# HKUNLP/efficient-attention

Hardware: AMD Instinct MI355X
Metric: attn fwd+bwd tokens/s per GPU at N=784, d=64; 1/2/4/8-GPU DDP scaling (higher is better)
Workload: dtype bf16; 1 GPU; lara attention layer fwd+bwd+SGD, x=[128,28,28,192] per GPU (N=784, h=3, d=64), bf16 autocast; attn=lara, global_batch=128, seq_len=784, heads=3, head_dim=64, parallelism=dp1, hipgraph=True, gemm_tunableop=False

## Files before the change

efficient-attention_amd/build.py:

```python
#!/usr/bin/env python3
import glob
import os
import subprocess
import sys

HERE = os.path.dirname(os.path.abspath(__file__))
CSRC = os.path.join(HERE, "csrc")
LIBDIR = os.path.join(HERE, "lib")
INCLUDE = os.path.join(os.path.dirname(HERE), "include")
HIPCC = os.environ.get("HIPCC", "/opt/rocm/bin/hipcc")
FLAGS = ["--offload-arch=gfx950", "-O3", "-std=c++17", "-fPIC", "-mllvm", "-amdgpu-mfma-vgpr-form", "-I" + INCLUDE, "-I" + CSRC]

LIB_SOURCES = ["ea_capi.hip", "ea_window_fwd.hip", "ea_window_bwd.hip", "ea_eva_landmark.hip",
               "ea_lara_x.hip", "ea_lara_y.hip", "ea_lara_f.hip", "ea_softmax.hip",
               "ea_lara_merge.hip", "ea_proj.hip", "ea_lara_segment.hip",
               "ea_rows_mlp.hip", "ea_wgrad.hip", "ea_linear.hip", "ea_lmk2.hip", "ea_scatter.hip", "ea_proj_rs.hip",
               "ea_performer_f32.hip", "ea_fold.hip", "ea_lara_seglin.hip", "ea_layernorm.hip", "ea_dgrad_rs.hip", "ea_f32_attn.hip",
               "ea_kernelized.hip", "ea_ceva_decode.hip", "ea_ceva_decode_linear.hip", "ea_ceva_decode_vocab.hip", "ea_lara_xp.hip",
               "ea_vocab_score.hip", "ea_adaptive_score.hip", "ea_adaptive_pick.hip", "ea_vocab_nll.hip", "ea_adaptive_nll.hip"]


def _cuid(src):
    return "-cuid=" + os.path.splitext(src)[0]


def _newer(target, deps):
    if not os.path.exists(target):
        return True
    t = os.path.getmtime(target)
    return any(os.path.getmtime(d) > t for d in deps)


def _run(cmd):
    r = subprocess.run(cmd, stdout=subprocess.PIPE, stderr=subprocess.STDOUT, text=True)
    if r.returncode != 0:
        raise RuntimeError("build failed: %s\n%s" % (" ".join(cmd), r.stdout))
    return r.stdout


def build(force=False, verbose=False):
    os.makedirs(LIBDIR, exist_ok=True)
    headers = glob.glob(os.path.join(CSRC, "*.h")) + glob.glob(os.path.join(INCLUDE, "*.h"))
    objs, jobs = [], []
    for src in LIB_SOURCES:
        s = os.path.join(CSRC, src)
        o = os.path.join(LIBDIR, src.replace(".hip", ".o"))
        if force or _newer(o, [s] + headers):
            if verbose:
                print("hipcc -c", src, flush=True)
            jobs.append([HIPCC] + FLAGS + [_cuid(src), "-c", s, "-o", o])
        objs.append(o)
    if jobs:
# ... 55 lines not shown
```

efficient-attention_amd/csrc/ea_capi.hip:

```cpp
#include <stdlib.h>
#include <cmath>
#include "ea_window.h"
#include "ea_landmark_params.h"
#include "ea_lara.h"
#include "ea_softmax.h"
#include "ea_lara_lmk.h"
#include "ea_lara_merge.h"
#include "ea_layernorm.h"
#include "ea_lara_segment.h"
#include "ea_scatter.h"
#include "ea_rows_mlp.h"
#include "ea_performer_f32.h"
#include "ea_kernelized.h"
#include "ea_f32_tile.h"
#include "ea_f32_attn.h"
#include "ea_linear.h"
#include "ea_proj.h"
#include "ea_fold.h"
#include "ea_lara_seglin.h"

using namespace ea;

static bool t4_ok32(const ea_t4* t, int D, int N) {
  return view_ok(t, D, 2) && (int64_t)N * t->sn < ((int64_t)1 << 31);
// ... 1326 lines not shown
  if ((dpq == nullptr) != (dpk == nullptr)) return EA_E_BADARG;
  if (dpq && (pool_r <= 0 || gh % pool_r || gw % pool_r)) return EA_E_BADARG;
  if (uq && (!qkv || !qbar || !lse_t || ldq < 192 || (ldq & 7) || C <= 0)) return EA_E_BADARG;
  if (uq && C > 64) return EA_E_UNSUPPORTED;
  if (!uq && !dpq) return EA_E_BADARG;
  if ((int64_t)B * gh * gw >= ((int64_t)1 << 31)) return EA_E_BADARG;
  return dgrad_fin_launch(dtype, dqkv, (long)ldy, qkv, (long)ldq, w, w_f32, dx, dx_f32, (long)ldx, B, gh, gw, pool_r, C, scale,
                          qbar, uq, lse_t, dpq, dpk, (hipStream_t)stream);
}

int32_t ea_linear_pool_supported(int32_t in_features, int32_t out_features, int32_t B, int32_t gh, int32_t gw, int32_t r) {
  return proj_rs_pool_supported(in_features, out_features, B, gh, gw, r);
}

int ea_linear_w32_pool(int32_t dtype, int32_t B, int32_t gh, int32_t gw, int32_t r, int32_t in_features, int32_t out_features,
                       const void* a, int32_t a_f32, int64_t lda, const float* w, const float* bias, void* y, int64_t ldy,
                       void* a_cast, float* pooled_q, float* pooled_k, void* w_cast, void* stream) {
  if (!a || !w || !y || !pooled_q || !pooled_k || ((uintptr_t)a & 15) || ((uintptr_t)w & 15) || ((uintptr_t)y & 15) ||
      ((uintptr_t)bias & 15) || ((uintptr_t)a_cast & 15) || ((uintptr_t)pooled_q & 15) || ((uintptr_t)pooled_k & 15) ||
      ((uintptr_t)w_cast & 15))
    return EA_E_BADARG;
  if (lda < in_features || ldy < out_features || (lda & 7) || (ldy & 7)) return EA_E_BADARG;
  if (!proj_rs_pool_supported(in_features, out_features, B, gh, gw, r)) return EA_E_UNSUPPORTED;
  return proj_rs_dispatch(dtype, a, a_f32, w, bias, y, a_cast, B * gh * gw, (long)lda, (long)ldy, (hipStream_t)stream, B, gh, gw,
                          r, pooled_q, pooled_k, w_cast, nullptr);
}

int ea_linear_w192_prepare(int32_t dtype, const float* wq, const float* wp, void* w16q, void* wq_sw, void* w16p, void* w16pT,
                           void* stream) {
  if (!wq || !w16q || !wq_sw || ((uintptr_t)wq & 15) || ((uintptr_t)wp & 15) || ((uintptr_t)w16q & 15) || ((uintptr_t)wq_sw & 15) ||
      ((uintptr_t)w16p & 15) || ((uintptr_t)w16pT & 15))
    return EA_E_BADARG;
  if (wp && (!w16p || !w16pT)) return EA_E_BADARG;
  return w192_prepare_dispatch(dtype, wq, wp, w16q, wq_sw, w16p, w16pT, nullptr, (hipStream_t)stream);
}

int ea_linear_w192_prepare_t(int32_t dtype, const float* wq, const float* wp, void* w16q, void* wq_sw, void* w16p, void* w16pT,
                             void* wqT_sw, void* stream) {
  if (!wq || !w16q || !wq_sw || !wqT_sw || ((uintptr_t)wq & 15) || ((uintptr_t)wp & 15) || ((uintptr_t)w16q & 15) ||
      ((uintptr_t)wq_sw & 15) || ((uintptr_t)w16p & 15) || ((uintptr_t)w16pT & 15) || ((uintptr_t)wqT_sw & 15))
    return EA_E_BADARG;
  if (wp && (!w16p || !w16pT)) return EA_E_BADARG;
  return w192_prepare_dispatch(dtype, wq, wp, w16q, wq_sw, w16p, w16pT, wqT_sw, (hipStream_t)stream);
}

int ea_linear_wsw(int32_t dtype, int32_t rows, int32_t B, int32_t gh, int32_t gw, int32_t r, const void* a, int32_t a_f32, int64_t lda,
                  const void* wq_sw, const float* bias, void* y, int64_t ldy, void* a_cast, float* pooled_q, float* pooled_k,
                  void* stream) {
  if (!a || !wq_sw || !y || ((uintptr_t)a & 15) || ((uintptr_t)wq_sw & 15) || ((uintptr_t)y & 15) || ((uintptr_t)bias & 15) ||
      ((uintptr_t)a_cast & 15) || ((uintptr_t)pooled_q & 15) || ((uintptr_t)pooled_k & 15))
    return EA_E_BADARG;
  if (lda < 192 || ldy < 576 || (lda & 7) || (ldy & 7) || rows <= 0) return EA_E_BADARG;
  if (r != 0) {
    if (!pooled_q || !pooled_k || rows != B * gh * gw) return EA_E_BADARG;
    if (!proj_rs_pool_supported(192, 576, B, gh, gw, r)) return EA_E_UNSUPPORTED;
  }
  return proj_rs_dispatch(dtype, a, a_f32, nullptr, bias, y, a_cast, rows, (long)lda, (long)ldy, (hipStream_t)stream, B, gh, gw, r,
                          r ? pooled_q : nullptr, r ? pooled_k : nullptr, nullptr, wq_sw);
}

}

static int fill_sb(const ea_sb_geom* g, SbP& p) {
  if (!g || g->B <= 0 || g->H <= 0 || g->N <= 0 || g->window <= 0 || (g->dtype != EA_BF16 && g->dtype != EA_F16))
    return EA_E_BADARG;
  if (g->D != 64 || g->M <= 0 || g->M > 64) return EA_E_UNSUPPORTED;
  p.B = g->B; p.H = g->H; p.N = g->N; p.M = g->M; p.w = g->window;
  p.G.N = g->N; p.G.attn2d = g->attn_2d; p.G.gh = g->attn_2d ? g->gh : 1; p.G.gw = g->attn_2d ? g->gw : g->N;
  if (g->attn_2d) {
    if (g->gh % g->window || g->gw % g->window || g->gh * g->gw != g->N) return EA_E_BADARG;
    p.Wq = g->window * g->window;
    p.nwin = (g->gh / g->window) * (g->gw / g->window);
  } else {
    if (g->N % g->window) return EA_E_BADARG;
    p.Wq = g->window;
    p.nwin = g->N / g->window;
// ... 1427 lines not shown
```

efficient-attention_amd/csrc/ea_linear.h:

```cpp
#pragma once
#include "ea_common.h"

namespace ea {

int linear_supported(int K, int NO);
int proj_rs_supported(int K, int NO);
int proj_rs_pool_supported(int K, int NO, int B, int gh, int gw, int r);
int proj_rs_dispatch(int dtype, const void* a, int a_f32, const float* w, const float* bias, void* y, void* a_cast, int rows,
                     long lda, long ldy, hipStream_t st, int B, int gh, int gw, int r, float* pq, float* pk, void* w_cast,
                     const void* wsw);
int w192_prepare_dispatch(int dtype, const float* wq, const float* wp, void* w16q, void* wsw, void* w16p, void* w16pT, void* wtsw,
                          hipStream_t st);
int dgrad_rs_supported(int K, int NO);
int dgrad_fin_launch(int dtype, const void* dqkv, long ldy, const void* qkv, long ldq, const void* w, int w_f32, void* dx, int dx_f32,
                     long ldx, int B, int gh, int gw, int pool_r, int C, float scale, const float* qbar, const float* uq,
                     const float* lse_t, const float* dpq, const float* dpk, hipStream_t st);
int dgrad_rs_dispatch(int dtype, const void* dy, const void* w, int w_f32, void* dx, int dx_f32, int rows, long ldy, long ldx,
                      hipStream_t st);
int linear_dispatch(int dtype, const void* a, int a_f32, const void* w, int w_mode, const float* bias, void* y, int y_f32,
                    void* a_cast, int rows, int K, int NO, long lda, long ldy, hipStream_t st);
int wgrad_slices(int rows, int M, int K);
int wgrad_pair_slices(int rows, int M1, int K1, int M2, int K2);
int wgrad_pair_dispatch(int dtype, int rows, const void* dy1, const void* x1, float* part1, float* db1, long ld1, int M1, int K1,
                        const void* dy2, const void* x2, float* part2, float* db2, long ld2, int M2, int K2, hipStream_t st);
int wgrad_dispatch(int dtype, const void* dy, const void* x, float* part, float* db_part, long part_ld, int rows, int M,
                   int K, hipStream_t st);
int part_sum_dispatch(const float* part, float* out, int S, int n, long ld, hipStream_t st);
int multi_sum_dispatch(int K, const float* const* part, const int* S, const int* n, const long long* ld, float* const* out,
                       hipStream_t st);

}
```

efficient-attention_amd/csrc/ea_proj_rs.hip:

```cpp
#include "ea_common.h"
#include "ea_linear.h"

namespace ea {

struct RsP {
  const char* a;
  const float* w;
  const float* bias;
  char* y;
  char* a_cast;
  char* w_cast;
  int rows, ntiles;
  long lda, ldy;
  float *pq, *pk;
  int gw, cw, Lc, ntok, ncell;
  unsigned m_Lc, m_cw;
  long long* prof;
  const char* wsw;
};

constexpr int RS_K = 192, RS_NO = 576, RS_WAVES = 12, RS_TOK = 32, RS_KT = RS_K / 32, RS_SLABS = RS_K / 64;

EA_DEV int rs_off(int slab, int tok, int chunk16) { return slab * (RS_TOK * 128) + lds_off3<64>(tok, chunk16); }

// ... 177 lines not shown
      const u32x4 o = {third[0][0], third[0][1], third[1][0], third[1][1]};
      stg16(p.y + ((size_t)tok * p.ldy + c0 + 32 + 8 * (g >> 1)) * 2, o);
    }
#ifndef EA_RS_NOPOOLMATH
    if constexpr (POOL > 0) {
      if (tprev >= 0) pool_out(tprev, buf ^ 1);
    }
#endif
  }
  EA_BLKX(p, 1);
  if constexpr (POOL > 0) {
    if (tprev >= 0) {
      __syncthreads();
      pool_out(tprev, buf ^ 1);
    }
  }
  EA_BLK(p, 1);
}

int proj_rs_supported(int K, int NO) { return K == RS_K && NO == RS_NO; }

static unsigned rs_magic(int d) { return (unsigned)((1ull << 32) / (unsigned)d) + 1u; }

int proj_rs_pool_supported(int K, int NO, int B, int gh, int gw, int r) {
  if (K != RS_K || NO != RS_NO || (r != 2 && r != 4) || B <= 0 || gh <= 0 || gw <= 0 || gh % r || gw % r) return 0;
  const long Lc = (long)(gh / r) * (gw / r), ncell = (long)B * Lc;
  return ncell * Lc < (1l << 32) && (long)B * gh * gw < (1l << 31);
}

template <typename E>
__global__ __launch_bounds__(256) void w192_prepare_kernel(const float* __restrict__ wq, const float* __restrict__ wp,
                                                            char* __restrict__ w16q, char* __restrict__ wsw,
                                                            char* __restrict__ w16p, char* __restrict__ w16pT,
                                                            char* __restrict__ wtsw) {
  constexpr int NQ = RS_WAVES * 3 * RS_KT * 64, NP = RS_K * RS_K / 8, NT = 12 * (RS_NO / 32) * 64;
  const int i = blockIdx.x * 256 + threadIdx.x;
  if (i < NQ) {
    const int lane = i & 63, pc = i >> 6, ks = pc % RS_KT, wj = pc / RS_KT, j = wj % 3, wave = wj / 3;
    const int g = lane >> 4, li = lane & 15;
    const size_t e = (size_t)rs_col(wave, j, li) * RS_K + ks * 32 + 8 * g;
    const f32x4 lo = *reinterpret_cast<const f32x4*>(wq + e), hi = *reinterpret_cast<const f32x4*>(wq + e + 4);
    const float f[8] = {lo[0], lo[1], lo[2], lo[3], hi[0], hi[1], hi[2], hi[3]};
    const u32x4 w8 = pack8<E>(f);
    stg16(wsw + (size_t)i * 16, w8);
    stg16(w16q + e * 2, w8);
  } else if (i < NQ + NP && wp) {
    const int k = i - NQ, row = k / (RS_K / 8), c = k - row * (RS_K / 8);
    const size_t e = (size_t)row * RS_K + c * 8;
    const f32x4 lo = *reinterpret_cast<const f32x4*>(wp + e), hi = *reinterpret_cast<const f32x4*>(wp + e + 4);
    const float f[8] = {lo[0], lo[1], lo[2], lo[3], hi[0], hi[1], hi[2], hi[3]};
    const u32x4 w8 = pack8<E>(f);
    stg16(w16p + e * 2, w8);
    uint16_t* t = reinterpret_cast<uint16_t*>(w16pT);
#pragma unroll
    for (int q = 0; q < 4; ++q) {
      t[(size_t)(c * 8 + 2 * q) * RS_K + row] = (uint16_t)(w8[q] & 0xffffu);
      t[(size_t)(c * 8 + 2 * q + 1) * RS_K + row] = (uint16_t)(w8[q] >> 16);
    }
  } else if (i >= NQ + NP && i < NQ + NP + NT && wtsw) {
    const int k = i - NQ - NP, lane = k & 63, pc = k >> 6, ks = pc % (RS_NO / 32), wave = pc / (RS_NO / 32);
    const int g = lane >> 4, li = lane & 15;
    const float* src = wq + (size_t)(32 * ks + 8 * g) * RS_K + 16 * wave + li;
    float f[8];
#pragma unroll
    for (int q = 0; q < 8; ++q) f[q] = src[(size_t)q * RS_K];
    stg16(wtsw + (size_t)k * 16, pack8<E>(f));
  }
}

int w192_prepare_dispatch(int dtype, const float* wq, const float* wp, void* w16q, void* wsw, void* w16p, void* w16pT,
                          void* wtsw, hipStream_t st) {
  const int N = RS_WAVES * 3 * RS_KT * 64 + RS_K * RS_K / 8 + (wtsw ? 12 * (RS_NO / 32) * 64 : 0);
  const dim3 g((N + 255) / 256), b(256);
  if (dtype == EA_BF16) hipLaunchKernelGGL(w192_prepare_kernel<BF16>, g, b, 0, st, wq, wp, (char*)w16q, (char*)wsw, (char*)w16p, (char*)w16pT, (char*)wtsw);
  else if (dtype == EA_F16) hipLaunchKernelGGL(w192_prepare_kernel<F16>, g, b, 0, st, wq, wp, (char*)w16q, (char*)wsw, (char*)w16p, (char*)w16pT, (char*)wtsw);
  else return EA_E_BADARG;
  return (int)hipGetLastError();
}

int proj_rs_dispatch(int dtype, const void* a, int a_f32, const float* w, const float* bias, void* y, void* a_cast, int rows,
                     long lda, long ldy, hipStream_t st, int B, int gh, int gw, int r, float* pq, float* pk, void* w_cast,
                     const void* wsw) {
  if (rows <= 0) return EA_OK;
  RsP p = {};
  p.a = (const char*)a; p.w = w; p.bias = bias; p.y = (char*)y; p.a_cast = a_f32 ? (char*)a_cast : nullptr;
  p.w_cast = wsw ? nullptr : (char*)w_cast;
  p.wsw = (const char*)wsw;
  p.rows = rows; p.ntiles = (rows + RS_TOK - 1) / RS_TOK; p.lda = lda; p.ldy = ldy;
  const int pool = r * r;
  if (pool) {
    if (!pq || !pk || rows != B * gh * gw) return EA_E_BADARG;
    p.pq = pq; p.pk = pk; p.gw = gw; p.cw = gw / r; p.Lc = (gh / r) * p.cw; p.ntok = gh * gw; p.ncell = B * p.Lc;
    p.m_Lc = rs_magic(p.Lc); p.m_cw = rs_magic(p.cw);
    p.ntiles = (p.ncell * pool + RS_TOK - 1) / RS_TOK;
  }
  int grid = ea_device_cus();
  if (grid > p.ntiles) grid = p.ntiles;
  const dim3 g((unsigned)grid), b(RS_WAVES * 64);
#ifdef EA_PROFILE
  ProfReport rep;
  p.prof = rep.arm(st, "proj_rs", pool);
#endif
#define EA_RS_LAUNCH2(E_, AF_, W_)                                                                             \
  do {                                                                                                         \
    if (pool == 16) hipLaunchKernelGGL((proj_rs_kernel<E_, AF_, 16, W_>), g, b, 0, st, p);                     \
    else if (pool == 4) hipLaunchKernelGGL((proj_rs_kernel<E_, AF_, 4, W_>), g, b, 0, st, p);                  \
    else hipLaunchKernelGGL((proj_rs_kernel<E_, AF_, 0, W_>), g, b, 0, st, p);                                 \
  } while (0)
// ... 21 lines not shown
```

efficient-attention_amd/efficient_attention/_native.py:

```python
import ctypes
import os

import torch

_HERE = os.path.dirname(os.path.abspath(__file__))
_LIB_PATH = os.environ.get(
    "EA_HIP_LIB", os.path.join(os.path.dirname(_HERE), "lib", "libea_hip.so"))

EA_BF16, EA_F16, EA_F32 = 0, 1, 2
_DTYPES = {torch.bfloat16: EA_BF16, torch.float16: EA_F16}


class ea_t4(ctypes.Structure):
    _fields_ = [("ptr", ctypes.c_void_p), ("sb", ctypes.c_int64), ("sh", ctypes.c_int64),
                ("sn", ctypes.c_int64)]


ABI_VERSION = 38


class ea_geom(ctypes.Structure):
    _fields_ = [("B", ctypes.c_int32), ("H", ctypes.c_int32), ("N", ctypes.c_int32),
                ("D", ctypes.c_int32), ("dtype", ctypes.c_int32), ("attn_2d", ctypes.c_int32),
                ("gh", ctypes.c_int32), ("gw", ctypes.c_int32), ("window", ctypes.c_int32),
# ... 115 lines not shown
    "ea_lara_landmarks_bwd_cb": [_MG] + [_P] * 23,
    "ea_lara_landmarks_saved_floats": [_MG],
    "ea_lara_merge_fwd": [_I] * 5 + [_P] * 8,
    "ea_lara_merge_bwd": [_I] * 5 + [_F] + [_P] * 16,
    "ea_bias_grad_parts": [_I, _I],
    "ea_bias_grad": [_I, _I, _I, _P, _P, _P, _P],
    "ea_colsum_f32": [_I, _I, _P, _P, _P],
    "ea_colsum2_f32": [_I, _I, _P, _P, _I, _P, _P, _P],
    "ea_slice_sum": [_I, _I, _I, _F, _P, _P, _P, _P],
    "ea_stream_copy": [_P, _P, _L, _P],
    "ea_lara_segment_fwd": [_G, _T, _T] + [_P] * 12,
    "ea_lara_segment_bwd": [_G, _T, _T] + [_P] * 11 + [_T, _T, _P, _P],
    "ea_lara_parts": [_LG],
    "ea_lara_stats_fwd": [_LG, _T, _T, _T, _P, _P, _P, _P, _P, _P],
    "ea_lara_out_fwd": [_LG, _T, _P, _P, _P, _P, _P, _P, _T, _P, _P, _P],
    "ea_lara_bwd_q": [_LG, _T, _T, _P, _P, _P, _P, _P, _P, _T, _P, _P, _P, _P, _P],
    "ea_lara_bwd_qstats": [_LG, _T, _T] + [_P] * 16,
    "ea_lara_bwd_k": [_LG, _T, _T, _P, _P, _P, _P, _P, _P, _T, _T, _P],
    "ea_lara_bwd_kstats": [_LG, _T, _T] + [_P] * 8,
    "ea_lara_bwd_qcorr": [_LG, _T, _P, _P, _P, _T, _P],
    "ea_lara_fused_parts": [_LG],
    "ea_lara_bwd_q_fused": [_LG, _T, _T, _P, _P, _P, _P, _P, _P, _P, _P, _T, _P, _P, _P, _P, _P, _P],
    "ea_lara_bwd_k_fused": [_LG, _T, _T, _P, _P, _P, _P, _P, _P, _T, _T, _P, _P],
    "ea_lara_bwd_finish": [_LG, _T, _P, _P, _P, _P, _P, _I, _I, _I, _T, _T, _P],
    "ea_lara_sample_fwd": [_I, _I, _I, _I, _I, _I, _F] + [_P] * 8,
    "ea_lara_sample_bwd": [_I, _I, _I, _I, _I, _I, _F] + [_P] * 10,
    "ea_adaptive_pool2d_fwd": [_I, _I, _I, _I, _I, _I, _I, _T, _P, _P],
    "ea_adaptive_pool2d_bwd": [_I, _I, _I, _I, _I, _I, _I, _P, _T, _P],
    "ea_gather_sum": [_I, _I, _I, _P, _P, _P, _P],
    "ea_table_bias_fwd": [_I, _I, _I, _I, _I, _F, _P, _P, _P, _P],
    "ea_multi_cast": [_I, _I, _P, _P, _P, _P],
    "ea_linear_w192_prepare": [_I, _P, _P, _P, _P, _P, _P, _P],
    "ea_linear_w192_prepare_t": [_I, _P, _P, _P, _P, _P, _P, _P, _P],
    "ea_linear_wsw": [_I, _I, _I, _I, _I, _I, _P, _I, _L, _P, _P, _P, _L, _P, _P, _P, _P],
    "ea_table_bias_bwd": [_I, _I, _I, _I, _I, _I, _F, _P, _P, _P, _P],
    "ea_linear_supported": [_I, _I],
    "ea_linear": [_I, _I, _I, _I, _P, _I, _L, _P, _P, _P, _I, _L, _P, _P],
    "ea_linear_w32": [_I, _I, _I, _I, _P, _I, _L, _P, _I, _P, _P, _I, _L, _P, _P],
    "ea_linear_pool_supported": [_I] * 6,
    "ea_f32_attn_fwd": [_FA, _T, _T, _T, _T, _T, _P, _P, _P, _P, _P, _P, _T, _P, _P, _P],
    "ea_f32_attn_bwd": [_FA, _T, _T, _T, _T, _T, _P, _P, _P, _P, _P, _P, _T, _T, _P, _P, _T, _P, _P, _P, _P, _P, _P],
    "ea_f32_gather_mean_fwd": [_I, _I, _I, _I, _I, _I, _T, _P, _P, _P, _P],
    "ea_f32_gather_mean_bwd": [_I, _I, _I, _I, _I, _I, _P, _P, _P, _P, _P],
    "ea_linear_dgrad_supported": [_I, _I],
    "ea_linear_dgrad": [_I, _I, _I, _I, _P, _L, _P, _I, _P, _I, _L, _P],
    "ea_linear_dgrad_finish": [_I, _I, _I, _I, _I, _I, _F, _P, _L, _P, _L, _P, _I, _P, _I, _L, _P, _P, _P, _P, _P, _P],
    "ea_linear_w32_pool": [_I] * 7 + [_P, _I, _L, _P, _P, _P, _L, _P, _P, _P, _P, _P],
    "ea_wgrad_parts": [_I, _I, _I],
    "ea_wgrad": [_I, _I, _I, _I, _P, _P, _P, _P, _L, _P],
    "ea_wgrad_pair_parts": [_I, _I, _I, _I, _I],
    "ea_layernorm_parts": [_I],
    "ea_layernorm_fwd": [_I, _I, _I, _P, _P, _P, _F, _P, _P, _P],
    "ea_layernorm_bwd": [_I, _I, _I, _P, _P, _P, _P, _P, _P, _P],
    "ea_wgrad_pair": [_I, _I, _I, _I, _P, _P, _P, _P, _L, _I, _I, _P, _P, _P, _P, _L, _P],
    "ea_part_sum": [_I, _I, _L, _P, _P, _P],
    "ea_multi_sum": [_I, _P, _P, _P, _P, _P, _P],
    "ea_lara_layer_plan": [_LL, ctypes.POINTER(ea_lara_layer_sizes)],
    "ea_lara_layer_fwd": [_LL, _T, _T, _T, _P, _P, _P, _T, _P, _P, _I, _P],
    "ea_lara_layer_fwd_proj": [_LL, _T, _T, _T, _P, _P, _P, _T, _P, _P, _I, _P, _P, _P, _L, _P],
    "ea_lara_layer_bwd": [_LL, _T, _T, _T, _P, _P, _P, _T, _T, _T, _T, _P, _P, _P, _I, _P],
    "ea_eva_layer_plan": [_EL, ctypes.POINTER(ea_eva_layer_sizes)],
    "ea_eva_layer_fwd": [_EL, _T, _T, _T, _P, _P, _P, _T, _P, _I, _P],
    "ea_eva_layer_bwd": [_EL, _T, _T, _T, _P, _P, _P, _T, _T, _T, _T, _T, _P, _P, _P, _P, _I, _P],
    "ea_scatter_parts": [_SG],
    "ea_scatter_kmax": [_SG, _T, _P, _P, _P, _P],
    "ea_scatter_kv": [_SG, _T, _T, _P, _P, _P, _P, _P, _P],
# ... 294 lines not shown
```

efficient-attention_amd/efficient_attention/_ops.py:

```python
import collections
import ctypes
import math
import os
import threading
import typing
import warnings

import torch
import torch.nn.functional as F

from . import _feature_cores as _fc
from . import _native as nv

KERNEL_TIMER = nv.KERNEL_TIMER
_DIRECT = os.environ.get("EA_DIRECT_IMPL", "1") == "1"


def _ea_op(name, impl, *args):
    if _DIRECT and not torch.compiler.is_compiling() and torch._C._len_torch_dispatch_stack() == 0:
        return impl(*args)
    return getattr(torch.ops.ea, name)(*args)


def landmark_flops(BH, L, C, D, has_mlp, mixed, eva, bwd):
# ... 1412 lines not shown

def project_qkv_pooled(x2, wq, bq32, cdtype, want_cast, B, H, W, r, pq, pk, w_cast=None):
    rows, K = x2.shape
    a_f32 = x2.dtype == torch.float32
    y = torch.empty((rows, 576), dtype=cdtype, device=x2.device)
    a_cast = torch.empty((rows, K), dtype=cdtype, device=x2.device) if (a_f32 and want_cast) else None
    label = "ea_linear_w32_pool"
    if nv.KERNEL_TIMER.enabled:
        label = "ea_linear[192->576,%s->16,+pool]" % ("f32" if a_f32 else "16")
        _note_bytes(label, rows * (K * x2.element_size() + 576 * 2 + (K * 2 if a_cast is not None else 0)))
    nv.call_as(label, "ea_linear_w32_pool", _ELEM[cdtype], B, H, W, r, K, 576, nv.ptr(x2), int(a_f32), x2.stride(0), nv.ptr(wq),
               nv.ptr(bq32), nv.ptr(y), 576, nv.ptr(a_cast), nv.ptr(pq), nv.ptr(pk), nv.ptr(w_cast), nv.stream())
    return y, a_cast


USE_W192 = os.environ.get("EA_W192_PREPARE", "1") == "1"


def w192_usable(wq, wp, cdtype):
    return (USE_W192 and _DIRECT and not torch.compiler.is_compiling() and torch._C._len_torch_dispatch_stack() == 0
            and cdtype in _ELEM and wq.is_cuda and wq.dtype == torch.float32 and wp.dtype == torch.float32
            and tuple(wq.shape) == (576, 192) and tuple(wp.shape) == (192, 192) and wq.is_contiguous() and wp.is_contiguous()
            and (wq.storage_offset() * 4) % 16 == 0 and (wp.storage_offset() * 4) % 16 == 0)


def prepare_w192(wq, wp, cdtype):
    return _prepare_w192(wq, wp, cdtype, False)


def prepare_w192_t(wq, wp, cdtype):
    return _prepare_w192(wq, wp, cdtype, True)


def _prepare_w192(wq, wp, cdtype, with_t):
    dev = wq.device
    w16q = torch.empty((576, 192), dtype=cdtype, device=dev)
    wsw = torch.empty((576 * 192,), dtype=cdtype, device=dev)
    w16p = torch.empty((192, 192), dtype=cdtype, device=dev)
    w16pT = torch.empty((192, 192), dtype=cdtype, device=dev)
    if not with_t:
        nv.call("ea_linear_w192_prepare", _ELEM[cdtype], nv.ptr(wq.detach()), nv.ptr(wp.detach()), nv.ptr(w16q), nv.ptr(wsw),
                nv.ptr(w16p), nv.ptr(w16pT), nv.stream())
        return w16q, wsw, w16p, w16pT
    wtsw = torch.empty((576 * 192,), dtype=cdtype, device=dev)
    nv.call("ea_linear_w192_prepare_t", _ELEM[cdtype], nv.ptr(wq.detach()), nv.ptr(wp.detach()), nv.ptr(w16q), nv.ptr(wsw),
            nv.ptr(w16p), nv.ptr(w16pT), nv.ptr(wtsw), nv.stream())
    return w16q, wsw, w16p, w16pT, wtsw


def project_qkv_wsw(x2, wsw, w16q, bq32, cdtype, want_cast, grid=None, pq=None, pk=None):
    rows, K = x2.shape
    a_f32 = x2.dtype == torch.float32
    if grid is None and rows < 65536:
        y, ac = ea_linear(x2, w16q, bq32, cdtype, want_cast)
        return y, ac
    y = torch.empty((rows, 576), dtype=cdtype, device=x2.device)
    a_cast = torch.empty((rows, K), dtype=cdtype, device=x2.device) if (a_f32 and want_cast) else None
    B, H, W, r = grid if grid is not None else (0, 0, 0, 0)
    label = "ea_linear_wsw"
    if nv.KERNEL_TIMER.enabled:
        label = "ea_linear[192->576,%s->16%s]" % ("f32" if a_f32 else "16", ",+pool" if grid is not None else "")
        _note_bytes(label, rows * (K * x2.element_size() + 576 * 2 + (K * 2 if a_cast is not None else 0)))
    nv.call_as(label, "ea_linear_wsw", _ELEM[cdtype], rows, B, H, W, r, nv.ptr(x2), int(a_f32), x2.stride(0), nv.ptr(wsw),
               nv.ptr(bq32), nv.ptr(y), 576, nv.ptr(a_cast), nv.ptr(pq), nv.ptr(pk), nv.stream())
    return y, a_cast

# ... 226 lines not shown
    def bwd(self, dout, qkv5, out, saved, defer, fin_ok):
        saved, params = saved[:self.nsaved], saved[self.nsaved:]
        head = (dout, qkv5, self.mask_u8, self.noise, list(saved))
        if not defer:
            g = _ea_op("lara_bwd", lara_bwd_impl, *head, *self.lists, list(params))
            return g[0], g[1:], (), None
        use_fin = bool(fin_ok and self.cfg.dup == 0 and self.cfg.L <= 64)
        g = _lara_backward(*head, self.cfg, list(params), defer_param_sums=True, defer_finish=use_fin)
        fin = (g.finish, qkv5.view(qkv5.shape[0] * qkv5.shape[1], -1)) if use_fin else None
        return g.dqkv, g.params or [], g.partials, fin

    def scatter(self, res, extra):
        return _mlp_grads(res["mlp_W"][0], res["mlp_v"][0], self.dims[2]) if "mlp_W" in res else extra


class CoreModuleFn(torch.autograd.Function):

    @staticmethod
    def forward(ctx, x, wq, bq, wp, bp, core, cdtype, heads, *inputs):
        B, C = x.shape[0], x.shape[-1]
        N = x.numel() // (B * C)
        d = C // heads
        x2 = x.reshape(-1, C)
        elem = _ELEM[cdtype]
        need = ctx.needs_input_grad
        direct = _DIRECT and not torch.compiler.is_compiling() and torch._C._len_torch_dispatch_stack() == 0
        lin = linear_w32_impl if direct else torch.ops.ea.linear_w32
        core.setup(B, N, heads, d, elem, inputs, any(need))
        bq32 = None if bq is None else (bq if bq.dtype == torch.float32 else bq.float())
        bp32 = None if bp is None else (bp if bp.dtype == torch.float32 else bp.float())
        want = x2.dtype == torch.float32 and need[1]
        lib = module_proj_lib(C)
        w16q = w16p = b16p = None
        w192 = prepare_w192_t(wq, wp, cdtype) if (not lib and w192_usable(wq, wp, cdtype)) else None
        w16pT = None if w192 is None else w192[3]
        if lib:
            w16q, b16q, w16p, b16p = lib_casts(wq, bq, wp, bp, cdtype)
            y, xc = lib_project(x2, wq, bq32, w16q, b16q, cdtype)
            want = True
        else:
            done = core.project(x2, wq, bq32, cdtype, want, need[0], w192) if direct else None
            if done is not None:
                y, xc, w16q = done
            elif w192 is not None:
                w16q = w192[0]
                y, xc = project_qkv_wsw(x2, w192[1], w16q, bq32, cdtype, want)
            else:
                y, xc = lin(x2, wq, bq32, elem, False, False, want)
        xl = x2 if x2.dtype == cdtype else (xc if want else None)
        qkv5 = y.view(B, N, 3, heads, d)
        done = core.fwd_project(qkv5, inputs, w192[2], bp32, cdtype) if (direct and w192 is not None) else None
        if done is not None:
            out, y2, saved = done
        else:
            out, saved = core.fwd(qkv5, inputs)
        o2 = out.reshape(-1, C)
        if done is not None:
            pass
        elif lib:
            with torch.autocast(device_type="cuda", enabled=False):
                y2 = F.linear(o2, w16p, b16p)
        elif w192 is not None:
            y2 = ea_linear(o2, w192[2], bp32, cdtype)[0]
        else:
            y2 = lin(o2, wp, bp32, elem, False, False, False)[0]
        wqT = w192[4] if (w192 is not None and w16q is w192[0]) else None
        ctx.save_for_backward(xl, qkv5, o2, wq, wp, w16q, w16p, w16pT, wqT, *saved)
        ctx.core = core
        ctx.meta = (x.shape, x.dtype, cdtype, None if bq is None else bq.dtype, None if bp is None else bp.dtype, wq.dtype, wp.dtype,
                    heads, [None if t is None else t.dtype for t in inputs])
        return y2.view(x.shape)

    @staticmethod
    def backward(ctx, dy):
        xl, qkv5, o2, wq, wp, w16q, w16p, w16pT, wqT, *saved = ctx.saved_tensors
        xshape, xdtype, cdtype, bqd, bpd, wqd, wpd, heads, in_dtypes = ctx.meta
        core = ctx.core
        C = xshape[-1]
        d = C // heads
        need = ctx.needs_input_grad
        if need[1] and xl is None:
            raise RuntimeError("%s: the weight gradient was requested but the forward did not keep its input"
                               % ctx._forward_cls.__name__)
        direct = _DIRECT and not torch.compiler.is_compiling() and torch._C._len_torch_dispatch_stack() == 0
        dy2 = dy.reshape(-1, C)
        if dy2.dtype != cdtype:
            dy2 = dy2.to(cdtype)
        if w16p is not None:
            dy2 = dy2 if dy2.is_contiguous() else dy2.contiguous()
            d_o2 = dy2 @ w16p
        elif w16pT is not None and _lin_rows_ok(dy2, cdtype):
            d_o2 = ea_linear(dy2, w16pT, None, cdtype)[0]
        else:
            lin = linear_w32_impl if direct else torch.ops.ea.linear_w32
            d_o2 = lin(dy2, wp, None, _ELEM[cdtype], True, False, False)[0]
        defer = direct and USE_MULTI_SUM
        need_bq, need_bp = bqd is not None and need[2], bpd is not None and need[4]
        qkv2 = qkv5.view(-1, 3 * C)
        pair = bool(defer and need[1] and need[3] and wgrad_pair_usable(qkv2, xl, dy2, o2))
        dwq = dbq = dwp = dbp = dx = None
        pend = []
        if need[3] and not pair:
            r_ = wgrad(dy2, o2, need_bp, defer=defer)
            if defer:
                pend.append(("proj", r_[0], r_[1]))
            else:
                dwp, dbp = r_[0].to(wpd), (r_[1].to(bpd) if need_bp else None)
        elif need_bp and not pair:
            dbp = bias_grad(dy2 if dy2.is_contiguous() else dy2.contiguous()).to(bpd)
        B, N = qkv5.shape[:2]
        dout, out = d_o2.view(B, N, heads, d), o2.view(B, N, heads, d)
        dqkv5, extra, parts, fin = core.bwd(dout, qkv5, out, saved, defer,
                                            bool(need[0] and dgrad_finish_usable(qkv2, wq, xdtype, heads, d)))
        pend += parts
        dqkv2 = dqkv5.view(-1, 3 * C)
        if fin is not None:
            dx = qkv_dgrad_finish(dqkv2, fin[1], wq, w16q, xdtype, fin[0], wqT).view(xshape)
        if pair:
            rq, rp = wgrad_pair(dqkv2, xl, need_bq, dy2, o2, need_bp)
            pend += [("qkv", rq[0], rq[1]), ("proj", rp[0], rp[1])]
        elif need[1]:
            r_ = wgrad(dqkv2, xl, need_bq, defer=defer)
            if defer:
# ... 1144 lines not shown
```

include/ea_hip.h:

```cpp
#ifndef EA_HIP_H
#define EA_HIP_H

#include <stdint.h>

#ifdef __cplusplus
extern "C" {
#endif

#define EA_BF16 0
#define EA_F16  1
#define EA_F32  2

#define EA_OK            0
#define EA_E_BADARG     -1
#define EA_E_UNSUPPORTED -2

typedef struct {
  void*   ptr;
  int64_t sb, sh, sn;
} ea_t4;

typedef struct {
  int32_t B, H, N, D;
  int32_t dtype;
// ... 607 lines not shown
int ea_adaptive_beam_c(int32_t M, int32_t C, int32_t n_tails, const int64_t* cutoffs, const int32_t* dims, const void* x,
                       int32_t x_dtype, int64_t ldx, const void* head, int32_t w_dtype, const void* const* proj,
                       const void* const* tables, void* ws, int64_t ws_bytes, int32_t W, int32_t eos, int32_t max_new,
                       float* score, int32_t* t, int32_t* nfin, int32_t* done, int64_t* token, int64_t* parent,
                       int32_t* hist_tok, int32_t* hist_par, float* fin_score, int32_t* fin_len, int32_t* fin_beam,
                       int32_t* cand_idx, float* cand_score, int32_t min_len, int32_t ngram, const int32_t* ban_tokens,
                       int32_t n_ban_tokens, const int32_t* prompt_tok, int32_t prompt_cap, const int32_t* prompt_len,
                       int32_t* gen, void* stream);

#define EA_VOCAB_NLL_BUDGET 268435456
int32_t ea_vocab_nll_chunk(int32_t M, int32_t V);
int64_t ea_vocab_nll_ws(int32_t M, int32_t K, int32_t V, int32_t chunk_cols);
int ea_vocab_nll_grad(int32_t M, int32_t K, int32_t V, const void* x, int32_t x_dtype, int64_t ldx, const void* w,
                      int32_t w_dtype, const int64_t* targets, const float* lse, const float* d, int32_t v0, int32_t Vc,
                      void* g, int64_t ldg, void* gt, int64_t ldm, void* stream);
int ea_gemm_nt16(int32_t M, int32_t N, int32_t K, const void* a, int64_t lda, const void* b, int64_t ldb, int32_t dtype,
                 float* out, int64_t ldo, int32_t accumulate, void* stream);

int64_t ea_adaptive_nll_ws(int32_t M, int32_t C, int32_t n_tails, const int64_t* cutoffs, const int32_t* dims,
                           int32_t chunk_cols);
int ea_vocab_nll_grad_rows(int32_t M, int32_t K, int32_t V, const void* x, int32_t x_dtype, int64_t ldx, const void* w,
                           int32_t w_dtype, const int64_t* targets, const float* lse, const float* d, int32_t v0, int32_t Vc,
                           void* g, int64_t ldg, void* gt, int64_t ldm, const int32_t* trows, const int32_t* count,
                           int64_t target_base, void* stream);
int ea_gemm_nt16_rows(int32_t M, int32_t N, int32_t K, const void* a, int64_t lda, const void* b, int64_t ldb, int32_t dtype,
                      float* out, int64_t ldo, int32_t accumulate, const int32_t* orows, const int32_t* count, void* stream);
int ea_rows_transpose16(int32_t M, int32_t K, const void* src, int32_t src_dtype, int64_t ld, const int32_t* rows,
                        const int32_t* count, void* out, int32_t out_dtype, int64_t ldm, void* stream);
int ea_adaptive_score_masked(int32_t M, int32_t C, int32_t n_tails, const int64_t* cutoffs, const int32_t* dims, const void* x,
                             int32_t x_dtype, int64_t ldx, const int64_t* targets, const void* head, int32_t w_dtype,
                             const void* const* proj, const void* const* tables, const void* const* hmask, void* ws,
                             int64_t ws_bytes, float* logp, int64_t* token_head, void* stream);

#ifdef __cplusplus
}
#endif
#endif
```

Measured before the change: 213.4 million tokens/s.

## Add register-resident-weight 192x192 linear kernel for output projection fwd and dgrad

Adds a persistent kernel for 192->192 linears. Each wave keeps its slice of a pre-swizzled weight image in registers while token tiles stream through double-buffered LDS with prefetch. The weight-prepare kernel now also emits the swizzled images for the projection weight and its transpose, and the lara module uses the new kernel for the forward output projection and the backward input gradient. The aim is to cut weight reloads and per-tile overhead compared with the generic ea_linear path, at the cost of a larger prepare kernel and one more saved tensor.

```diff
diff --git a/efficient-attention_amd/build.py b/efficient-attention_amd/build.py
--- a/efficient-attention_amd/build.py
+++ b/efficient-attention_amd/build.py
@@ -17,7 +17,8 @@
                "ea_rows_mlp.hip", "ea_wgrad.hip", "ea_linear.hip", "ea_lmk2.hip", "ea_scatter.hip", "ea_proj_rs.hip",
                "ea_performer_f32.hip", "ea_fold.hip", "ea_lara_seglin.hip", "ea_layernorm.hip", "ea_dgrad_rs.hip", "ea_f32_attn.hip",
                "ea_kernelized.hip", "ea_ceva_decode.hip", "ea_ceva_decode_linear.hip", "ea_ceva_decode_vocab.hip", "ea_lara_xp.hip",
-               "ea_vocab_score.hip", "ea_adaptive_score.hip", "ea_adaptive_pick.hip", "ea_vocab_nll.hip", "ea_adaptive_nll.hip"]
+               "ea_vocab_score.hip", "ea_adaptive_score.hip", "ea_adaptive_pick.hip", "ea_vocab_nll.hip", "ea_adaptive_nll.hip",
+               "ea_linear_rs192.hip"]
 
 
 def _cuid(src):
diff --git a/efficient-attention_amd/csrc/ea_capi.hip b/efficient-attention_amd/csrc/ea_capi.hip
--- a/efficient-attention_amd/csrc/ea_capi.hip
+++ b/efficient-attention_amd/csrc/ea_capi.hip
@@ -1382,7 +1382,7 @@
       ((uintptr_t)w16p & 15) || ((uintptr_t)w16pT & 15))
     return EA_E_BADARG;
   if (wp && (!w16p || !w16pT)) return EA_E_BADARG;
-  return w192_prepare_dispatch(dtype, wq, wp, w16q, wq_sw, w16p, w16pT, nullptr, (hipStream_t)stream);
+  return w192_prepare_dispatch(dtype, wq, wp, w16q, wq_sw, w16p, w16pT, nullptr, nullptr, nullptr, (hipStream_t)stream);
 }
 
 int ea_linear_w192_prepare_t(int32_t dtype, const float* wq, const float* wp, void* w16q, void* wq_sw, void* w16p, void* w16pT,
@@ -1391,7 +1391,26 @@
       ((uintptr_t)wq_sw & 15) || ((uintptr_t)w16p & 15) || ((uintptr_t)w16pT & 15) || ((uintptr_t)wqT_sw & 15))
     return EA_E_BADARG;
   if (wp && (!w16p || !w16pT)) return EA_E_BADARG;
-  return w192_prepare_dispatch(dtype, wq, wp, w16q, wq_sw, w16p, w16pT, wqT_sw, (hipStream_t)stream);
+  return w192_prepare_dispatch(dtype, wq, wp, w16q, wq_sw, w16p, w16pT, wqT_sw, nullptr, nullptr, (hipStream_t)stream);
+}
+
+int ea_linear_w192_prepare_rs(int32_t dtype, const float* wq, const float* wp, void* w16q, void* wq_sw, void* w16p, void* w16pT,
+                              void* wqT_sw, void* wp_rs, void* wpT_rs, void* stream) {
+  if (!wq || !wp || !w16q || !wq_sw || !w16p || !w16pT || !wqT_sw || !wp_rs || !wpT_rs) return EA_E_BADARG;
+  if (((uintptr_t)wq & 15) || ((uintptr_t)wp & 15) || ((uintptr_t)w16q & 15) || ((uintptr_t)wq_sw & 15) || ((uintptr_t)w16p & 15) ||
+      ((uintptr_t)w16pT & 15) || ((uintptr_t)wqT_sw & 15) || ((uintptr_t)wp_rs & 15) || ((uintptr_t)wpT_rs & 15))
+    return EA_E_BADARG;
+  return w192_prepare_dispatch(dtype, wq, wp, w16q, wq_sw, w16p, w16pT, wqT_sw, wp_rs, wpT_rs, (hipStream_t)stream);
+}
+
+int ea_linear_rs192(int32_t dtype, const void* a, int64_t lda, const void* image, const float* bias, void* y, int64_t ldy,
+                    int32_t rows, void* stream) {
+  if (dtype != EA_BF16 && dtype != EA_F16) return EA_E_BADARG;
+  if (rows <= 0) return EA_OK;
+  if (!a || !image || !y) return EA_E_BADARG;
+  if (((uintptr_t)a & 15) || ((uintptr_t)image & 15) || ((uintptr_t)y & 15) || ((uintptr_t)bias & 15)) return EA_E_UNSUPPORTED;
+  if (!linear_rs192_supported(rows, (long)lda, (long)ldy)) return EA_E_UNSUPPORTED;
+  return linear_rs192_dispatch(dtype, a, (long)lda, image, bias, y, (long)ldy, rows, (hipStream_t)stream);
 }
 
 int ea_linear_wsw(int32_t dtype, int32_t rows, int32_t B, int32_t gh, int32_t gw, int32_t r, const void* a, int32_t a_f32, int64_t lda,
diff --git a/efficient-attention_amd/csrc/ea_linear.h b/efficient-attention_amd/csrc/ea_linear.h
--- a/efficient-attention_amd/csrc/ea_linear.h
+++ b/efficient-attention_amd/csrc/ea_linear.h
@@ -10,6 +10,10 @@
                      long lda, long ldy, hipStream_t st, int B, int gh, int gw, int r, float* pq, float* pk, void* w_cast,
                      const void* wsw);
 int w192_prepare_dispatch(int dtype, const float* wq, const float* wp, void* w16q, void* wsw, void* w16p, void* w16pT, void* wtsw,
+                          void* wp_rs, void* wpT_rs, hipStream_t st);
+constexpr int rs192_row(int pair, int j, int li) { return 32 * pair + 8 * (li >> 2) + (li & 3) + 4 * j; }
+int linear_rs192_supported(int rows, long lda, long ldy);
+int linear_rs192_dispatch(int dtype, const void* a, long lda, const void* wimg, const float* bias, void* y, long ldy, int rows,
                           hipStream_t st);
 int dgrad_rs_supported(int K, int NO);
 int dgrad_fin_launch(int dtype, const void* dqkv, long ldy, const void* qkv, long ldq, const void* w, int w_f32, void* dx, int dx_f32,
diff --git a/efficient-attention_amd/csrc/ea_linear_rs192.hip b/efficient-attention_amd/csrc/ea_linear_rs192.hip
--- /dev/null
+++ b/efficient-attention_amd/csrc/ea_linear_rs192.hip
@@ -0,0 +1,91 @@
+#include "ea_common.h"
+#include "ea_linear.h"
+
+namespace ea {
+
+struct Rs192P {
+  const char* a;
+  const char* wimg;
+  const float* bias;
+  char* y;
+  int rows, ntiles;
+  long lda, ldy;
+};
+
+constexpr int R1_K = 192, R1_WAVES = 12, R1_KT = R1_K / 32, R1_SLABS = R1_K / 64, R1_CPR = R1_K / 8;
+
+template <typename E>
+__global__ __launch_bounds__(R1_WAVES * 64, 1) void lin_rs192_kernel(const Rs192P p) {
+  constexpr int TOK = 32, SLAB = TOK * 128;
+  __shared__ __attribute__((aligned(16))) char tile[2][R1_SLABS * SLAB];
+  __shared__ __attribute__((aligned(16))) float bias_s[R1_K];
+  const int tid = threadIdx.x, lane = tid & 63, g = lane >> 4, li = lane & 15;
+  const int wave = __builtin_amdgcn_readfirstlane(tid >> 6);
+  const int pair = wave >> 1, half = wave & 1;
+  const int st_tok = tid / R1_CPR, st_c = tid - st_tok * R1_CPR;
+  u32x4 nb;
+  auto issue = [&](int t) {
+    const int tok = min(t * TOK + st_tok, p.rows - 1);
+    nb = ldg16(p.a + (size_t)tok * p.lda * 2 + st_c * 16);
+  };
+  int t = blockIdx.x;
+  issue(t);
+  typename E::x8 wr[2][R1_KT];
+#pragma unroll
+  for (int j = 0; j < 2; ++j)
+#pragma unroll
+    for (int ks = 0; ks < R1_KT; ++ks)
+      wr[j][ks] = as_x8<E>(ldg16(p.wimg + ((size_t)((pair * 2 + j) * R1_KT + ks) * 64 + lane) * 16));
+  for (int i = tid; i < R1_K; i += R1_WAVES * 64) bias_s[i] = p.bias ? E::to_f(E::from_f(p.bias[i])) : 0.f;
+  const int st_off = (st_c >> 3) * SLAB + lds_off3<64>(st_tok, st_c & 7);
+  const int rd_off = lds_off3<64>(16 * half + li, g);
+
+#pragma unroll
+  for (int j = 0; j < 2; ++j)
+#pragma unroll
+    for (int ks = 0; ks < R1_KT; ++ks) asm volatile("" ::"v"(wr[j][ks]));
+  int buf = 0;
+  for (; t < p.ntiles; t += gridDim.x, buf ^= 1) {
+    sts16(tile[buf] + st_off, nb);
+    issue(t + gridDim.x);
+    __syncthreads();
+    f32x4 acc0 = f32x4{0.f, 0.f, 0.f, 0.f}, acc1 = acc0;
+#pragma unroll
+    for (int ks = 0; ks < R1_KT; ++ks) {
+      const typename E::x8 b = as_x8<E>(lds16(tile[buf] + (ks >> 1) * SLAB + (rd_off ^ ((ks & 1) << 6))));
+      acc0 = E::mma(wr[0][ks], b, acc0);
+      acc1 = E::mma(wr[1][ks], b, acc1);
+    }
+    const int n = 32 * pair + 8 * g;
+    const f32x4 b0 = *reinterpret_cast<const f32x4*>(bias_s + n), b1 = *reinterpret_cast<const f32x4*>(bias_s + n + 4);
+    const int tok = min(t * TOK + 16 * half + li, p.rows - 1);
+    const f32x4 v0 = acc0 + b0, v1 = acc1 + b1;
+    u32x4 o;
+    o[0] = pack2<E>(v0[0], v0[1]); o[1] = pack2<E>(v0[2], v0[3]);
+    o[2] = pack2<E>(v1[0], v1[1]); o[3] = pack2<E>(v1[2], v1[3]);
+    stg16(p.y + ((size_t)tok * p.ldy + n) * 2, o);
+  }
+}
+
+int linear_rs192_supported(int rows, long lda, long ldy) {
+  return rows > 0 && lda >= R1_K && ldy >= R1_K && !(lda & 7) && !(ldy & 7) && (long)rows * (lda > ldy ? lda : ldy) < (1l << 40) &&
+         rows <= (1 << 30);
+}
+
+int linear_rs192_dispatch(int dtype, const void* a, long lda, const void* wimg, const float* bias, void* y, long ldy, int rows,
+                          hipStream_t st) {
+  if (rows <= 0) return EA_OK;
+  if (!linear_rs192_supported(rows, lda, ldy)) return EA_E_UNSUPPORTED;
+  if (dtype != EA_BF16 && dtype != EA_F16) return EA_E_BADARG;
+  Rs192P p;
+  p.a = (const char*)a; p.wimg = (const char*)wimg; p.bias = bias; p.y = (char*)y;
+  p.rows = rows; p.ntiles = (rows + 31) / 32; p.lda = lda; p.ldy = ldy;
+  int grid = ea_device_cus();
+  if (grid > p.ntiles) grid = p.ntiles;
+  const dim3 gr((unsigned)grid), b(R1_WAVES * 64);
+  if (dtype == EA_BF16) hipLaunchKernelGGL(lin_rs192_kernel<BF16>, gr, b, 0, st, p);
+  else hipLaunchKernelGGL(lin_rs192_kernel<F16>, gr, b, 0, st, p);
+  return (int)hipGetLastError();
+}
+
+}
diff --git a/efficient-attention_amd/csrc/ea_proj_rs.hip b/efficient-attention_amd/csrc/ea_proj_rs.hip
--- a/efficient-attention_amd/csrc/ea_proj_rs.hip
+++ b/efficient-attention_amd/csrc/ea_proj_rs.hip
@@ -233,7 +233,8 @@
 __global__ __launch_bounds__(256) void w192_prepare_kernel(const float* __restrict__ wq, const float* __restrict__ wp,
                                                             char* __restrict__ w16q, char* __restrict__ wsw,
                                                             char* __restrict__ w16p, char* __restrict__ w16pT,
-                                                            char* __restrict__ wtsw) {
+                                                            char* __restrict__ wtsw, char* __restrict__ wp_rs,
+                                                            char* __restrict__ wpT_rs) {
   constexpr int NQ = RS_WAVES * 3 * RS_KT * 64, NP = RS_K * RS_K / 8, NT = 12 * (RS_NO / 32) * 64;
   const int i = blockIdx.x * 256 + threadIdx.x;
   if (i < NQ) {
@@ -252,6 +253,10 @@
     const float f[8] = {lo[0], lo[1], lo[2], lo[3], hi[0], hi[1], hi[2], hi[3]};
     const u32x4 w8 = pack8<E>(f);
     stg16(w16p + e * 2, w8);
+    if (wp_rs) {
+      const int r = row & 31, li = 4 * (r >> 3) + (r & 3);
+      stg16(wp_rs + ((size_t)(((row >> 5) * 2 + ((r >> 2) & 1)) * RS_KT + (c >> 2)) * 64 + 16 * (c & 3) + li) * 16, w8);
+    }
     uint16_t* t = reinterpret_cast<uint16_t*>(w16pT);
 #pragma unroll
     for (int q = 0; q < 4; ++q) {
@@ -266,15 +271,24 @@
 #pragma unroll
     for (int q = 0; q < 8; ++q) f[q] = src[(size_t)q * RS_K];
     stg16(wtsw + (size_t)k * 16, pack8<E>(f));
+  } else if (i >= NQ + NP + NT && i < NQ + NP + NT + NP && wpT_rs) {
+    const int k = i - NQ - NP - NT, lane = k & 63, pc = k >> 6, ks = pc % RS_KT, pj = pc / RS_KT;
+    const int g = lane >> 4, li = lane & 15;
+    const float* src = wp + (size_t)(32 * ks + 8 * g) * RS_K + rs192_row(pj >> 1, pj & 1, li);
+    float f[8];
+#pragma unroll
+    for (int q = 0; q < 8; ++q) f[q] = src[(size_t)q * RS_K];
+    stg16(wpT_rs + (size_t)k * 16, pack8<E>(f));
   }
 }
 
 int w192_prepare_dispatch(int dtype, const float* wq, const float* wp, void* w16q, void* wsw, void* w16p, void* w16pT,
-                          void* wtsw, hipStream_t st) {
-  const int N = RS_WAVES * 3 * RS_KT * 64 + RS_K * RS_K / 8 + (wtsw ? 12 * (RS_NO / 32) * 64 : 0);
+                          void* wtsw, void* wp_rs, void* wpT_rs, hipStream_t st) {
+  const int N = RS_WAVES * 3 * RS_KT * 64 + RS_K * RS_K / 8 + ((wtsw || wpT_rs) ? 12 * (RS_NO / 32) * 64 : 0) +
+                (wpT_rs ? RS_K * RS_K / 8 : 0);
   const dim3 g((N + 255) / 256), b(256);
-  if (dtype == EA_BF16) hipLaunchKernelGGL(w192_prepare_kernel<BF16>, g, b, 0, st, wq, wp, (char*)w16q, (char*)wsw, (char*)w16p, (char*)w16pT, (char*)wtsw);
-  else if (dtype == EA_F16) hipLaunchKernelGGL(w192_prepare_kernel<F16>, g, b, 0, st, wq, wp, (char*)w16q, (char*)wsw, (char*)w16p, (char*)w16pT, (char*)wtsw);
+  if (dtype == EA_BF16) hipLaunchKernelGGL(w192_prepare_kernel<BF16>, g, b, 0, st, wq, wp, (char*)w16q, (char*)wsw, (char*)w16p, (char*)w16pT, (char*)wtsw, (char*)wp_rs, (char*)wpT_rs);
+  else if (dtype == EA_F16) hipLaunchKernelGGL(w192_prepare_kernel<F16>, g, b, 0, st, wq, wp, (char*)w16q, (char*)wsw, (char*)w16p, (char*)w16pT, (char*)wtsw, (char*)wp_rs, (char*)wpT_rs);
   else return EA_E_BADARG;
   return (int)hipGetLastError();
 }
diff --git a/efficient-attention_amd/efficient_attention/_native.py b/efficient-attention_amd/efficient_attention/_native.py
--- a/efficient-attention_amd/efficient_attention/_native.py
+++ b/efficient-attention_amd/efficient_attention/_native.py
@@ -171,6 +171,8 @@
     "ea_multi_cast": [_I, _I, _P, _P, _P, _P],
     "ea_linear_w192_prepare": [_I, _P, _P, _P, _P, _P, _P, _P],
     "ea_linear_w192_prepare_t": [_I, _P, _P, _P, _P, _P, _P, _P, _P],
+    "ea_linear_w192_prepare_rs": [_I] + [_P] * 10,
+    "ea_linear_rs192": [_I, _P, _L, _P, _P, _P, _L, _I, _P],
     "ea_linear_wsw": [_I, _I, _I, _I, _I, _I, _P, _I, _L, _P, _P, _P, _L, _P, _P, _P, _P],
     "ea_table_bias_bwd": [_I, _I, _I, _I, _I, _I, _F, _P, _P, _P, _P],
     "ea_linear_supported": [_I, _I],
diff --git a/efficient-attention_amd/efficient_attention/_ops.py b/efficient-attention_amd/efficient_attention/_ops.py
--- a/efficient-attention_amd/efficient_attention/_ops.py
+++ b/efficient-attention_amd/efficient_attention/_ops.py
@@ -1468,6 +1468,38 @@
     return _prepare_w192(wq, wp, cdtype, True)
 
 
+USE_LIN_RS192 = os.environ.get("EA_LIN_RS192", "1") == "1"
+
+
+def prepare_w192_rs(wq, wp, cdtype):
+    if not USE_LIN_RS192:
+        return _prepare_w192(wq, wp, cdtype, True) + (None, None)
+    dev = wq.device
+    w16q = torch.empty((576, 192), dtype=cdtype, device=dev)
+    wsw = torch.empty((576 * 192,), dtype=cdtype, device=dev)
+    wtsw = torch.empty((576 * 192,), dtype=cdtype, device=dev)
+    w16p, w16pT, wp_rs, wpT_rs = torch.empty((4, 192, 192), dtype=cdtype, device=dev).unbind(0)
+    nv.call("ea_linear_w192_prepare_rs", _ELEM[cdtype], nv.ptr(wq.detach()), nv.ptr(wp.detach()), nv.ptr(w16q), nv.ptr(wsw),
+            nv.ptr(w16p), nv.ptr(w16pT), nv.ptr(wtsw), nv.ptr(wp_rs), nv.ptr(wpT_rs), nv.stream())
+    return w16q, wsw, w16p, w16pT, wtsw, wp_rs.view(-1), wpT_rs.view(-1)
+
+
+def _rs192_rows_ok(a2, cdtype):
+    return a2.dtype == cdtype and _lin_rows_ok(a2, cdtype) and a2.shape[1] == 192 and a2.stride(0) >= 192
+
+
+def linear_rs192(a2, image, bias32, cdtype):
+    rows = a2.shape[0]
+    y = torch.empty((rows, 192), dtype=cdtype, device=a2.device)
+    label = "ea_linear_rs192"
+    if nv.KERNEL_TIMER.enabled:
+        label = "ea_linear_rs192[192->192,16->16]"
+        _note_bytes(label, rows * (192 * 2 + 192 * 2))
+    nv.call_as(label, "ea_linear_rs192", _ELEM[cdtype], nv.ptr(a2), a2.stride(0), nv.ptr(image), nv.ptr(bias32), nv.ptr(y), 192,
+               rows, nv.stream())
+    return y
+
+
 def _prepare_w192(wq, wp, cdtype, with_t):
     dev = wq.device
     w16q = torch.empty((576, 192), dtype=cdtype, device=dev)
@@ -1760,8 +1792,9 @@
         want = x2.dtype == torch.float32 and need[1]
         lib = module_proj_lib(C)
         w16q = w16p = b16p = None
-        w192 = prepare_w192_t(wq, wp, cdtype) if (not lib and w192_usable(wq, wp, cdtype)) else None
+        w192 = prepare_w192_rs(wq, wp, cdtype) if (not lib and w192_usable(wq, wp, cdtype)) else None
         w16pT = None if w192 is None else w192[3]
+        wpT_rs = None if w192 is None else w192[6]
         if lib:
             w16q, b16q, w16p, b16p = lib_casts(wq, bq, wp, bp, cdtype)
             y, xc = lib_project(x2, wq, bq32, w16q, b16q, cdtype)
@@ -1788,12 +1821,14 @@
         elif lib:
             with torch.autocast(device_type="cuda", enabled=False):
                 y2 = F.linear(o2, w16p, b16p)
+        elif w192 is not None and w192[5] is not None and _rs192_rows_ok(o2, cdtype):
+            y2 = linear_rs192(o2, w192[5], bp32, cdtype)
         elif w192 is not None:
             y2 = ea_linear(o2, w192[2], bp32, cdtype)[0]
         else:
             y2 = lin(o2, wp, bp32, elem, False, False, False)[0]
         wqT = w192[4] if (w192 is not None and w16q is w192[0]) else None
-        ctx.save_for_backward(xl, qkv5, o2, wq, wp, w16q, w16p, w16pT, wqT, *saved)
+        ctx.save_for_backward(xl, qkv5, o2, wq, wp, w16q, w16p, w16pT, wqT, wpT_rs, *saved)
         ctx.core = core
         ctx.meta = (x.shape, x.dtype, cdtype, None if bq is None else bq.dtype, None if bp is None else bp.dtype, wq.dtype, wp.dtype,
                     heads, [None if t is None else t.dtype for t in inputs])
@@ -1801,7 +1836,7 @@
 
     @staticmethod
     def backward(ctx, dy):
-        xl, qkv5, o2, wq, wp, w16q, w16p, w16pT, wqT, *saved = ctx.saved_tensors
+        xl, qkv5, o2, wq, wp, w16q, w16p, w16pT, wqT, wpT_rs, *saved = ctx.saved_tensors
         xshape, xdtype, cdtype, bqd, bpd, wqd, wpd, heads, in_dtypes = ctx.meta
         core = ctx.core
         C = xshape[-1]
@@ -1817,6 +1852,8 @@
         if w16p is not None:
             dy2 = dy2 if dy2.is_contiguous() else dy2.contiguous()
             d_o2 = dy2 @ w16p
+        elif wpT_rs is not None and _rs192_rows_ok(dy2, cdtype):
+            d_o2 = linear_rs192(dy2, wpT_rs, None, cdtype)
         elif w16pT is not None and _lin_rows_ok(dy2, cdtype):
             d_o2 = ea_linear(dy2, w16pT, None, cdtype)[0]
         else:
diff --git a/include/ea_hip.h b/include/ea_hip.h
--- a/include/ea_hip.h
+++ b/include/ea_hip.h
@@ -663,6 +663,11 @@
                              const void* const* proj, const void* const* tables, const void* const* hmask, void* ws,
                              int64_t ws_bytes, float* logp, int64_t* token_head, void* stream);
 
+int ea_linear_rs192(int32_t dtype, const void* a, int64_t lda, const void* image, const float* bias, void* y, int64_t ldy,
+                    int32_t rows, void* stream);
+int ea_linear_w192_prepare_rs(int32_t dtype, const float* wq, const float* wp, void* w16q, void* wq_sw, void* w16p, void* w16pT,
+                              void* wqT_sw, void* wp_rs, void* wpT_rs, void* stream);
+
 #ifdef __cplusplus
 }
 #endif
```

New measurement: 217.3 million tokens/s, median of 6. 1.8% higher.
